# RaikoPipe/panda-gym

Hardware: AMD Instinct MI355X
Metric: aggregate env-steps/s, PandaReach 4096 envs @1 GPU; 1/2/4/8-GPU scaling (higher is better)
Workload: dtype f32; 1 GPU; PandaReach-v3 (ee control, sparse reward), 4096 envs per GPU, the reference's scene: table / plane contacts of the robot (BASELINE configs[1]); envs_per_gpu=4096, global_envs=4096, parallelism=env-sharded x1

## Files before the change

### panda-gym_amd/csrc/pgx_kernels.hip

```cpp
#include <hip/hip_runtime.h>
#include <math.h>
#include <stdint.h>

#include "../../include/pgx.h"
#include "pgx_default_model.h"
#include "pgx_common.h"
#include "pgx_dev.h"
#include "pgx_model_consts.h"
#include "pgx_rows.h"

#ifdef PGX_PROF
#define PGX_PROF_N 24
__device__ unsigned long long pgx_prof_counters[PGX_PROF_N];
#define PGX_PROF_WAVES 16384
__device__ unsigned long long pgx_prof_wave[PGX_PROF_WAVES][10];
extern "C" int pgx_prof_wave_read(unsigned long long* out, int n) {
    return (int)hipMemcpyFromSymbol(out, HIP_SYMBOL(pgx_prof_wave), sizeof(unsigned long long) * 10 * (size_t)n);
}
extern "C" int pgx_prof_read(unsigned long long* out, int clear) {
    hipError_t e = hipMemcpyFromSymbol(out, HIP_SYMBOL(pgx_prof_counters), sizeof(unsigned long long) * PGX_PROF_N);
    if (e == hipSuccess && clear) {
        unsigned long long z[PGX_PROF_N] = {0};
        e = hipMemcpyToSymbol(HIP_SYMBOL(pgx_prof_counters), z, sizeof z);
    }
// ... 287 lines not shown
}

__device__ __forceinline__ void mat_to_quat(const M3& M, float* q) {
    const float* m = M.m;
    float tr = m[0] + m[4] + m[8];
    if (tr > 0.0f) {
        float s = fast_sqrt(tr + 1.0f);
        q[3] = s * 0.5f;
        s = 0.5f * fast_rcp(s);
        q[0] = (m[7] - m[5]) * s;
        q[1] = (m[2] - m[6]) * s;
        q[2] = (m[3] - m[1]) * s;
    } else if (!(m[0] < m[4]) && !(m[0] < m[8])) {
        float s = fast_sqrt(m[0] - m[4] - m[8] + 1.0f);
        q[0] = s * 0.5f;
        s = 0.5f * fast_rcp(s);
        q[3] = (m[7] - m[5]) * s;
        q[1] = (m[3] + m[1]) * s;
        q[2] = (m[6] + m[2]) * s;
    } else if (m[0] < m[4] && !(m[4] < m[8])) {
        float s = fast_sqrt(m[4] - m[8] - m[0] + 1.0f);
        q[1] = s * 0.5f;
        s = 0.5f * fast_rcp(s);
        q[3] = (m[2] - m[6]) * s;
        q[2] = (m[7] + m[5]) * s;
        q[0] = (m[1] + m[3]) * s;
    } else {
        float s = fast_sqrt(m[8] - m[0] - m[4] + 1.0f);
        q[2] = s * 0.5f;
        s = 0.5f * fast_rcp(s);
        q[3] = (m[3] - m[1]) * s;
        q[0] = (m[2] + m[6]) * s;
        q[1] = (m[5] + m[7]) * s;
    }
}

__device__ __forceinline__ void chol7(float A[NJ][NJ]) {
#pragma unroll
    for (int j = 0; j < NJ; j++) {
        float s = A[j][j];
#pragma unroll
        for (int k = 0; k < j; k++) s -= A[j][k] * A[j][k];
        float inv = __builtin_amdgcn_rsqf(fmaxf(s, 1e-30f));
        A[j][j] = inv;
#pragma unroll
        for (int i = j + 1; i < NJ; i++) {
            float t = A[i][j];
#pragma unroll
            for (int k = 0; k < j; k++) t -= A[i][k] * A[j][k];
            A[i][j] = t * inv;
        }
    }
}
__device__ __forceinline__ void chol7_solve(const float L[NJ][NJ], const float* b, float* x) {
    float y[NJ];
#pragma unroll
    for (int i = 0; i < NJ; i++) {
        float s = b[i];
#pragma unroll
        for (int k = 0; k < i; k++) s -= L[i][k] * y[k];
        y[i] = s * L[i][i];
    }
#pragma unroll
    for (int i = NJ - 1; i >= 0; i--) {
        float s = y[i];
#pragma unroll
        for (int k = i + 1; k < NJ; k++) s -= L[k][i] * x[k];
        x[i] = s * L[i][i];
    }
}

template <bool PAR = false>
__device__ __forceinline__ void ik(MPtr mp, const float* q0, V3 target, const float* torn, float* qout) {
    float qs[NJ];
#pragma unroll
    for (int j = 0; j < NJ; j++) qs[j] = q0[j];
    float diff = 1e30f;
    const int max_iters = mp->ik_max_iters;
    const float residual = mp->ik_residual;
    for (int it = 0; it < max_iters; it++) {
        if (!(diff > residual)) break;
        PGX_PROF_COUNT(17, 1);
        MRef m = *fresh(mp);
        Chain k;
        fk_chain<PAR>(m, qs, k);
        V3 x = k.o[6] + mulc(k.R[6], kEePivot);
        M3 Ree = mulm(k.R[6], kEeRot);
        float cq[4], dq[4];
        mat_to_quat(Ree, cq);
        {
            const float ax = torn[0], ay = torn[1], az = torn[2], aw = torn[3];
            const float bx = -cq[0], by = -cq[1], bz = -cq[2], bw = cq[3];
            dq[0] = aw * bx + ax * bw + ay * bz - az * by;
            dq[1] = aw * by + ay * bw + az * bx - ax * bz;
            dq[2] = aw * bz + az * bw + ax * by - ay * bx;
            dq[3] = aw * bw - ax * bx - ay * by - az * bz;
        }
        float vn = fast_sqrt(dq[0] * dq[0] + dq[1] * dq[1] + dq[2] * dq[2]);
        float angle = 2.0f * atan2f(vn, dq[3]);
        if (angle > 3.14159265358979f) angle -= 6.28318530717959f;
        V3 axis = vn > 1e-30f ? (1.0f / vn) * v3(dq[0], dq[1], dq[2]) : v3(1.0f, 0.0f, 0.0f);
        V3 ep = target - x;
        V3 er = angle * axis;
        float A[NJ][NJ], g[NJ], dth[NJ];
        if constexpr (PAR) {
            V3 zs[NJ], os[NJ];
#pragma unroll
            for (int j = 0; j < NJ; j++) { zs[j] = col(k.R[j], 2); os[j] = k.o[j]; }
            const V3 jwc = pick_v3(zs), jvc = cross(jwc, x - pick_v3(os));
            const float gc = dot(jvc, ep) + dot(jwc, er);
            float Ac[NJ];
            sfor<0, NJ>([&](auto bc) __attribute__((always_inline)) {
                constexpr int b = decltype(bc)::value;
                const V3 jvb = v3(bcast16<b>(jvc.x), bcast16<b>(jvc.y), bcast16<b>(jvc.z));
                const V3 jwb = v3(bcast16<b>(jwc.x), bcast16<b>(jwc.y), bcast16<b>(jwc.z));
                Ac[b] = dot(jvc, jvb) + dot(jwc, jwb);
            });
            sfor<0, NJ>([&](auto ac) __attribute__((always_inline)) {
                constexpr int a = decltype(ac)::value;
                g[a] = bcast16<a>(gc);
                sfor<0, a + 1>([&](auto bc) __attribute__((always_inline)) {
                    constexpr int b = decltype(bc)::value;
                    A[a][b] = bcast16<a>(Ac[b]);
                });
                A[a][a] += m.ik_damping;
            });
        } else {
            V3 jv[NJ], jw[NJ];
#pragma unroll
            for (int j = 0; j < NJ; j++) {
                jw[j] = col(k.R[j], 2);
                jv[j] = cross(jw[j], x - k.o[j]);
            }
#pragma unroll
            for (int a = 0; a < NJ; a++) {
                g[a] = dot(jv[a], ep) + dot(jw[a], er);
#pragma unroll
                for (int b = 0; b <= a; b++) A[a][b] = dot(jv[a], jv[b]) + dot(jw[a], jw[b]);
                A[a][a] += m.ik_damping;
            }
        }
        chol7(A);
        chol7_solve(A, g, dth);
        float mx = 0.0f;
#pragma unroll
        for (int j = 0; j < NJ; j++) mx = fmaxf(mx, fabsf(dth[j]));
        float sc = mx > m.ik_max_angle ? m.ik_max_angle * fast_rcp(mx) : 1.0f;
#pragma unroll
        for (int j = 0; j < NJ; j++) qs[j] += dth[j] * sc;
        diff = norm(x - target);
    }
#pragma unroll
    for (int j = 0; j < NJ; j++) qout[j] = qs[j];
}

constexpr int AO_N = PGX_AO_OBSTACLES;
constexpr float kAoSize = 0.05f, kAoMargin = 0.001f;
constexpr float kAoCubeBound = 0.0866025404f;

__host__ __device__ constexpr int ao_slot(int c) {
    return kCapLink[c] < 0 ? -1 : (kCapLink[c] <= 7 ? kCapLink[c] : (kCapLink[c] == 9 ? 8 : -1));
}
__device__ constexpr int kAoSlot[PGX_NCAP] = {ao_slot(0), ao_slot(1), ao_slot(2), ao_slot(3), ao_slot(4),
                                              ao_slot(5), ao_slot(6), ao_slot(7), ao_slot(8), ao_slot(9),
                                              ao_slot(10), ao_slot(11), ao_slot(12), ao_slot(13)};
static_assert(PGX_NCAP == 14, "kAoSlot table");


__device__ __forceinline__ float box_sd(V3 P, V3 c, V3 h) {
    const float dx = fabsf(P.x - c.x) - h.x, dy = fabsf(P.y - c.y) - h.y, dz = fabsf(P.z - c.z) - h.z;
    const float ox = fmaxf(dx, 0.0f), oy = fmaxf(dy, 0.0f), oz = fmaxf(dz, 0.0f);
    return fast_sqrt(ox * ox + oy * oy + oz * oz) + fminf(fmaxf(dx, fmaxf(dy, dz)), 0.0f);
}

__device__ __forceinline__ V3 seg_closest(V3 A, V3 B, V3 C) {
    const V3 ab = B - A;
    const float l2 = dot(ab, ab);
    float t = l2 > 0.0f ? dot(C - A, ab) * fast_rcp(l2) : 0.0f;
    t = fminf(fmaxf(t, 0.0f), 1.0f);
    return A + t * ab;
}

__device__ __forceinline__ bool seg_meets_box(V3 A, V3 ab, V3 lo, V3 hi) {
    float t0 = 0.0f, t1 = 1.0f;
    bool miss = false;
    const float a[3] = {A.x, A.y, A.z}, d[3] = {ab.x, ab.y, ab.z}, l[3] = {lo.x, lo.y, lo.z}, u[3] = {hi.x, hi.y, hi.z};
#pragma unroll
    for (int i = 0; i < 3; i++) {
        if (fabsf(d[i]) < 1e-20f) {
            miss = miss || a[i] < l[i] || a[i] > u[i];
        } else {
            const float inv = fast_rcp(d[i]);
            const float ta = (l[i] - a[i]) * inv, tb = (u[i] - a[i]) * inv;
            t0 = fmaxf(t0, fminf(ta, tb));
            t1 = fminf(t1, fmaxf(ta, tb));
        }
// ... 1371 lines not shown
                sort_g1_by_depth(*Lp, es);
                wm = __builtin_amdgcn_readfirstlane(wm);
                while (wm) {
                    const int cn = __builtin_ctz(wm);
                    wm &= wm - 1u;
                    object_candidates_g(e, cap_tau<TAU_OBJ>(m, cn), *Lp, es, ob, Rc, cn, c, ((rm >> cn) & 1u) != 0);
                }
                PGX_PROF_MARK(21);
                sort_groups(*Lp, es);
            }
        }
    }
    PGX_PROF_MARK(1);
    const V3 g = v3(m.gravity[0], m.gravity[1], m.gravity[2]);
    const V3 base = v3(m.base[0], m.base[1], m.base[2]);
    const V3 zl = col(Rl, 2);
    const V3 ob_l = ol - base;
    const V3 cw = ol + mul(Rl, v3(K.com[0], K.com[1], K.com[2]));
    const V3 cb = cw - base;

    const float qdl = pick_arm(qd, 0.0f);
    const V3 t1 = qdl * zl;
    const V3 w = row_pre(t1);
    const V3 alt = cross(w - t1, t1);
    const V3 al = row_pre(alt);
    const V3 S = row_pre(cross(t1, ob_l));
    const V3 u = cross(w, ob_l) - S;
    const V3 dS = row_pre(cross(alt, ob_l) + cross(t1, u));
    const V3 v = cross(w, cb) - S;
    const V3 a = cross(al, cb) + cross(w, v) - dS;
    const S3 Iw = rot_sym_r(Rl, K.I);
    const V3 Iww = mul(Iw, w);
    const float wn = norm(w);
    const V3 Iow = mul(Rl, mul_sym(K.Iown, mul_t(Rl, w)));
    V3 F = K.mass * (a - g);
    V3 T = mul(Iw, al) + cross(w, Iww) + (m.ang_damp + m.ang_damp * wn) * Iow;
    {
        const V3 Fd = (K.mass * (m.lin_damp + m.lin_damp * norm(v))) * v;
        V3 Fg = v3(0, 0, 0), Tg = v3(0, 0, 0);
#pragma unroll
        for (int b = 0; b < PGX_NDAMP; b++) {
            const V3 rb = mulc(Rl, kDpos[b]);
            const V3 vb = u + cross(w, rb);
            const V3 fd = (kDmass[b] * (m.lin_damp + m.lin_damp * norm(vb))) * vb;
            Fg = Fg + fd;
            Tg = Tg + cross(ol + rb - cw, fd);
        }
        F = F + v3(lane_sel<NJ - 1>(Fg.x, Fd.x), lane_sel<NJ - 1>(Fg.y, Fd.y), lane_sel<NJ - 1>(Fg.z, Fd.z));
        T = T + v3(lane_sel<NJ - 1>(Tg.x, 0.0f), lane_sel<NJ - 1>(Tg.y, 0.0f), lane_sel<NJ - 1>(Tg.z, 0.0f));
    }
    const V3 Fs = row_suf(link_only(F));
    const V3 Ms = row_suf(link_only(T + cross(cb, F)));
    const float nbl = -dot(zl, Ms - cross(ob_l, Fs));
    float nb[NJ];
    sfor<0, NJ>([&](auto jc) __attribute__((always_inline)) {
        constexpr int j = decltype(jc)::value;
        nb[j] = bcast16<j>(nbl);
    });
    PGX_PROF_MARK(14);

    float Mt[NJ][NJ];
    {
        const float ml = link_only(K.mass);
        const S3 st = steiner(ml, cb);
        const float Mc = row_suf(ml);
        const V3 H = row_suf(ml * cb);
        const float Ixx = row_suf(link_only(Iw.xx + st.xx)), Iyy = row_suf(link_only(Iw.yy + st.yy));
        const float Izz = row_suf(link_only(Iw.zz + st.zz)), Ixy = row_suf(link_only(Iw.xy + st.xy));
        const float Ixz = row_suf(link_only(Iw.xz + st.xz)), Iyz = row_suf(link_only(Iw.yz + st.yz));
        const S3 Is = {Ixx, Iyy, Izz, Ixy, Ixz, Iyz};
        const V3 f = cross(zl, H - Mc * ob_l);
        const float Ho = dot(H, ob_l), oz = dot(ob_l, zl), Hz = dot(H, zl), oo = dot(ob_l, ob_l);
        const V3 n = mul(Is, zl) + (Mc * oo - 2.0f * Ho) * zl + oz * H + Hz * ob_l - (Mc * oz) * ob_l;
        float colv[NJ];
#pragma unroll
        for (int i = 0; i < NJ; i++) colv[i] = dot(z[i], n + cross(ol - o[i], f));
        sfor<0, NJ>([&](auto jc) __attribute__((always_inline)) {
            constexpr int j = decltype(jc)::value;
            sfor<0, j + 1>([&](auto ic) __attribute__((always_inline)) {
                constexpr int i = decltype(ic)::value;
                Mt[j][i] = bcast16<j>(colv[i]);
            });
        });
    }
    chol7(Mt);
    float (&vu)[NJ] = D.vu;
    {
        float qdd[NJ];
        chol7_solve(Mt, nb, qdd);
#pragma unroll
        for (int j = 0; j < NJ; j++) vu[j] = fminf(fmaxf(qd[j] + m.dt * qdd[j], -m.max_vel), m.max_vel);
    }

    PGX_PROF_MARK(15);
    {
        float y[NJ], x[NJ];
        sfor<0, NJ>([&](auto ic) __attribute__((always_inline)) {
            constexpr int i = decltype(ic)::value;
            float sacc = lane_sel<i>(1.0f, 0.0f);
#pragma unroll
            for (int k = 0; k < i; k++) sacc -= Mt[i][k] * y[k];
            y[i] = sacc * Mt[i][i];
        });
#pragma unroll
        for (int i = NJ - 1; i >= 0; i--) {
            float sacc = y[i];
#pragma unroll
            for (int k = i + 1; k < NJ; k++) sacc -= Mt[k][i] * x[k];
            x[i] = sacc * Mt[i][i];
        }
#pragma unroll
        for (int k = 0; k < NJ; k++) D.mcol[k] = x[k];
        sfor<0, NJ>([&](auto dc) __attribute__((always_inline)) {
            constexpr int d = decltype(dc)::value;
            D.mdiag[d] = bcast16<d>(x[d]);
        });
    }
    V3& vcu = D.vcu;
    V3& wcu = D.wcu;
    vcu = v3(0, 0, 0);
    wcu = v3(0, 0, 0);
    if (OBJ) {
        const float vn = norm(ob.v), wn2 = norm(ob.w);
        vcu = ob.v + m.dt * (g - (m.lin_damp + m.lin_damp * vn) * ob.v - cross(ob.w, ob.v));
        wcu = ob.w - (m.dt * (m.ang_damp + m.ang_damp * wn2)) * ob.w;
    }
}

__device__ __forceinline__ void object_integrate(MRef m, ObjState& ob, V3 v, V3 w) {
    ob.v = v;
    ob.w = w;
    ob.p = ob.p + m.dt * ob.v;
    float ang = norm(ob.w);
    if (ang * m.dt > 0.39269908f) ang = 0.39269908f * m.inv_dt;
    const float hdt = 0.5f * m.dt;
    const float f = ang < 0.001f ? (hdt - m.dt * m.dt * m.dt * 0.020833333333f * ang * ang)
                                 : __sinf(ang * hdt) * fast_rcp(ang);
    const float ax = ob.w.x * f, ay = ob.w.y * f, az = ob.w.z * f, aw = __cosf(ang * hdt);
    const float nx = aw * ob.qx + ax * ob.qw + ay * ob.qz - az * ob.qy;
    const float ny = aw * ob.qy + ay * ob.qw + az * ob.qx - ax * ob.qz;
    const float nz = aw * ob.qz + az * ob.qw + ax * ob.qy - ay * ob.qx;
    const float nw = aw * ob.qw - ax * ob.qx - ay * ob.qy - az * ob.qz;
// ... 392 lines not shown
            L.cache[8 + 2 * s + 1][ln] = s < n1 ? lam1[s][0] : 0.0f;
        }
    }
    if (OBJ) object_integrate(m, ob, vcu + dvl, wcu + dvw);
    PGX_PROF_MARK(5);
}

constexpr bool limit_rows_paired() {
    for (int r = 0; r < NJ; r++)
        if ((kPgxRowCode[r] >> 4) != 0) return false;
    for (int r = NJ; r + 1 < PGX_N_ROWS; r += 2)
        if ((kPgxRowCode[r] >> 4) != 1 || (kPgxRowCode[r + 1] >> 4) != 2 ||
            (kPgxRowCode[r] & 15) != (kPgxRowCode[r + 1] & 15))
            return false;
    return (PGX_N_ROWS - NJ) % 2 == 0;
}

constexpr int last_motor_row() {
    int r = 0;
    for (int i = 0; i < PGX_N_ROWS; i++)
        if ((kPgxRowCode[i] >> 4) == 0) r = i;
    return r;
}

template <int OBJ, int CONT, int PART = 1, int AO = 0, int FULL = 0>
__device__ __forceinline__ bool substep_g(MPtr mp, const PgxDevEnv& e, float* q, float* qd, const float* tq,
                                          ObjState& ob, ContactLdsGT<OBJ, FULL>* Lp, int es, int c, const LaneK& K,
                                          bool check = false) {
    MRef m = *fresh(mp);
    constexpr bool LDS_LIM = OBJ;
    constexpr bool NO_PART = OBJ && PART == 2;
    constexpr bool PERS = CONT && FULL && (OBJ || (AO && AO_PERS));
    Dyn D;
    substep_dyn_g<OBJ, CONT, AO, FULL>(m, e, q, qd, ob, Lp, es, D, c, K, check);
    if constexpr (AO) {
        if (D.coll) return true;
    }
    const V3 (&z)[NJ] = D.z;
    const V3 (&o)[NJ] = D.o;
    float vu[NJ];
#pragma unroll
    for (int j = 0; j < NJ; j++) vu[j] = D.vu[j];
    V3 vcu = D.vcu, wcu = D.wcu;
    PGX_PROF_MARK(2);
    const bool arm = c < NJ;
    const float inv_m = e.obj_inv_mass, inv_i = e.obj_inv_inertia;
    float mcol[NJ];
#pragma unroll
    for (int d = 0; d < NJ; d++) mcol[d] = D.mcol[d];
    const float kobj = OBJ ? ((c >= 7 && c < 10) ? inv_m : ((c >= 10 && c < 13) ? inv_i : 0.0f)) : 0.0f;
    const float vu_c = pick_gen(vu, vcu, wcu);
    float gv = 0.0f;

    constexpr int P0 = OBJ ? CG : 0;
    constexpr int CGR = ContactLdsGT<OBJ, FULL>::CGR;
    constexpr int NP = P0 + (CONT ? CGR : 0);
    constexpr int RB = CONT ? ContactLdsGT<OBJ, FULL>::RB : CGR;
    constexpr int NQR = ContactLdsGT<OBJ, FULL>::NQR;
    constexpr int NC_ = OBJ ? 13 : NJ;
    constexpr int XSTEP = 1;
    int n1x = 0;
    int nxr = 0;
    float cJ[NP > 0 ? NP : 1][3], cR[NP > 0 ? NP : 1][3], crhs[NP > 0 ? NP : 1][3], cjinv[NP > 0 ? NP : 1][3];
    float cden[NP > 0 ? NP : 1][3], clam[NP > 0 ? NP : 1][3];
    float pmu[NP > 0 ? NP : 1];
    bool act[NP > 0 ? NP : 1];
    int n0 = 0, n1 = 0;
    if (CONT) {
        ContactLdsGT<OBJ, FULL>& L = *Lp;
        n0 = L.cnt[0][es];
        n1 = L.cnt[1][es];
        const float erp_dt = m.contact_erp * m.inv_dt;
        float cid0[CG], cim0[CG], cid1[CGR], cim1[CGR];
#pragma unroll
        for (int s2 = 0; s2 < CG; s2++) {
            cid0[s2] = OBJ ? L.cache[2 * s2][es] : -1.0f;
            cim0[s2] = OBJ ? L.cache[2 * s2 + 1][es] : 0.0f;
        }
#pragma unroll
        for (int s2 = 0; s2 < CGR; s2++) {
            cid1[s2] = L.cache[CACHE1 + 2 * s2][es];
            cim1[s2] = L.cache[CACHE1 + 2 * s2 + 1][es];
        }
        auto warm_of = [&](const float* ids, const float* ims, auto n_c, float id) __attribute__((always_inline)) {
            float w = 0.0f;
#pragma unroll
            for (int s2 = 0; s2 < decltype(n_c)::value; s2++) w = ids[s2] == id ? m.warmstart * ims[s2] : w;
            return w;
        };
#pragma unroll
        for (int p = 0; p < NP; p++) pmu[p] = m.friction;
#pragma unroll
        for (int k = 0; k < P0; k++) {
            act[k] = k < n0;
            const float4 r4 = L.g0q[k][0][es];
            const V3 r = v3(r4.x, r4.y, r4.z);
            const float id = L.g0id[k][es];
            const float warm = warm_of(cid0, cim0, IC<CG>{}, id);
            V3 nk = lds3(L.g0n[k], es), t1, t2;
            nk = act[k] ? nk : v3(0.0f, 0.0f, 1.0f);
            plane_space(nk, t1, t2);
#pragma unroll
            for (int dir = 0; dir < 3; dir++) {
                const V3 lin = dir == 0 ? nk : (dir == 1 ? t1 : t2);
                const V3 ang = cross(r, lin);
                const float den = inv_m + dot(ang, ang) * inv_i;
                const float jinv = den > 2.220446e-16f ? fast_rcp(den) : 0.0f;
                const float rel = dot(lin, vcu) + dot(ang, wcu);
                float rhs;
                if (dir == 0) {
                    const float pen = L.g0d[k][es];
                    rhs = (pen > 0.0f ? (-rel - pen * m.inv_dt) : (-pen * erp_dt - rel)) * jinv;
                } else {
                    rhs = -rel * jinv;
                }
                const float J = pick_obj(lin, ang);
                cJ[k][dir] = act[k] ? J : 0.0f;
                cR[k][dir] = act[k] ? J * kobj : 0.0f;
                crhs[k][dir] = act[k] ? rhs : 0.0f;
                cjinv[k][dir] = act[k] ? jinv : 0.0f;
                cden[k][dir] = act[k] ? den : 0.0f;
                clam[k][dir] = (act[k] && dir == 0) ? warm : 0.0f;
                gv += cR[k][dir] * clam[k][dir];
            }
        }
        const V3 zc = pick_v3(z), oc = pick_v3(o);
        V3 gP[CGR], gN[CGR], gRb[CGR];
        int gJ[CGR], gW[CGR];
        float gId[CGR], gD[CGR];
        auto read_point = [&](int k) __attribute__((always_inline)) {
            gP[k] = v3(L.g1p[k][0][es], L.g1p[k][1][es], L.g1p[k][2][es]);
            gN[k] = v3(L.g1n[k][0][es], L.g1n[k][1][es], L.g1n[k][2][es]);
            gRb[k] = OBJ ? v3(L.g1rb[k][0][es], L.g1rb[k][1][es], L.g1rb[k][2][es]) : v3(0.0f, 0.0f, 0.0f);
            gJ[k] = L.g1j[k][es];
            gW[k] = PERS ? L.g1w[k][es] : -1;
            gId[k] = L.g1id[k][es];
            gD[k] = L.g1d[k][es];
        };
        auto warm_pt = [&](int w, float id) __attribute__((always_inline)) {
            return (PERS && w >= 0) ? m.warmstart * L.mimp[w < 0 ? 0 : w][es] : warm_of(cid1, cim1, IC<CGR>{}, id);
        };
        if (!AO && __any(n1 > 0)) {
#pragma unroll
            for (int k = 0; k < CGR; k++) read_point(k);
        }
#pragma unroll
        for (int k = 0; k < (CONT ? CGR : 0); k++) {
            const int p = P0 + k;
            act[p] = k < n1;
#pragma unroll
            for (int dir = 0; dir < 3; dir++) {
                cJ[p][dir] = 0.0f; cR[p][dir] = 0.0f; crhs[p][dir] = 0.0f;
                cjinv[p][dir] = 0.0f; cden[p][dir] = 0.0f; clam[p][dir] = 0.0f;
            }
            if (__any(act[p])) {
                if (AO) read_point(k);
                const V3 P = gP[k];
                const V3 n = gN[k];
                const V3 rb = gRb[k];
                const int jl = gJ[k];
                const float id = gId[k];
                pmu[p] = point_mu<AO, FULL>(m, id);
                const bool vs_obj = OBJ && id >= kTableIdLimit;
                const float warm = warm_pt(gW[k], id);
                V3 t1, t2;
                plane_space(n, t1, t2);
                const V3 Jv = (arm && c <= jl) ? cross(zc, P - oc) : v3(0, 0, 0);
#pragma unroll
                for (int dir = 0; dir < 3; dir++) {
                    const V3 u = dir == 0 ? n : (dir == 1 ? t1 : t2);
                    float J = dot(u, Jv);
                    if (OBJ) {
                        const V3 ca = cross(rb, u);
                        const float oj = pick_obj(-1.0f * u, -1.0f * ca);
                        J = (!arm && vs_obj) ? oj : J;
                    }
                    float R = kobj * J;
                    sfor<0, NJ>([&](auto bc) __attribute__((always_inline)) {
                        constexpr int b = decltype(bc)::value;
                        R += mcol[b] * bcast16<b>(J);
                    });
                    const float den = sum16(J * R);
                    const float rel = sum16(J * vu_c);
                    const float jinv = den > 2.220446e-16f ? fast_rcp(den) : 0.0f;
                    float rhs;
                    if (dir == 0) {
                        const float pen = gD[k];
                        rhs = (pen > 0.0f ? (-rel - pen * m.inv_dt) : (-pen * erp_dt - rel)) * jinv;
                    } else {
                        rhs = -rel * jinv;
                    }
                    cJ[p][dir] = act[p] ? J : 0.0f;
                    cR[p][dir] = act[p] ? R : 0.0f;
// ... 173 lines not shown
    PGX_PROF_MARK(23);

    float den[NJ], jinv[NJ];
#pragma unroll
    for (int d = 0; d < NJ; d++) {
        den[d] = D.mdiag[d];
        jinv[d] = den[d] > 2.220446e-16f ? fast_rcp(den[d]) : 0.0f;
    }
    float rhs[PGX_N_ROWS];
#pragma unroll
    for (int r = 0; r < PGX_N_ROWS; r++) {
        const int kind = kPgxRowCode[r] >> 4, d = kPgxRowCode[r] & 15;
        rhs[r] = 0.0f;
        if (kind == 0) {
            const float pos_term = (tq[d] - q[d]) * m.inv_dt;
            const float desired = m.kp * pos_term + vu[d] + m.kd * (0.0f - vu[d]);
            rhs[r] = desired - vu[d];
        }
    }
    auto init_limit_rows = [&]() __attribute__((always_inline)) {
#pragma unroll
        for (int r = 0; r < PGX_N_ROWS; r++) {
            const int kind = kPgxRowCode[r] >> 4, d = kPgxRowCode[r] & 15;
            if (kind == 0) continue;
            const float rel = kind == 2 ? -vu[d] : vu[d];
            const float pen = kind == 1 ? (q[d] - kLower[d]) : (kUpper[d] - q[d]);
            float verr = -rel, perr = 0.0f;
            if (pen > 0.0f) verr -= pen * m.inv_dt;
            else perr = -pen * m.erp * m.inv_dt;
            rhs[r] = perr + verr;
        }
    };
    bool ok_c = true;
    bool far_nc = true;
    if (arm) {
        float B = 0.0f;
#pragma unroll
        for (int k = 0; k < NJ; k++) B += fabsf(mcol[k]) * m.max_impulse[k];
        B = B * 1.001f + 1e-6f;
        float lo_a[NJ], up_a[NJ];
#pragma unroll
        for (int d = 0; d < NJ; d++) { lo_a[d] = kLower[d]; up_a[d] = kUpper[d]; }
        const float qc = pick_arm(q, 0.0f);
        const float penl = qc - pick_arm(lo_a, 0.0f), penu = pick_arm(up_a, 0.0f) - qc;
        ok_c = penl > 0.0f && penu > 0.0f && (vu_c - B) > -penl * m.inv_dt && (vu_c + B) < penu * m.inv_dt;
    }
    far_nc = !row_any(!ok_c);
    const bool far = far_nc && n1 == 0;
    float mcs[NJ], wms[NJ], wms2[NJ];
    constexpr int PK = AO ? PGX_PK_AO : PGX_PK;
    constexpr bool PKM = WROWS && (PK & 1) != 0, PKC = WROWS && (PK & 2) != 0;
    constexpr bool PKD = TWO && FULL && !PKM && !PKC && (PK & 4) != 0;
    constexpr bool MERGE = WROWS && !OBJ && !AO && !PKM && !PKC && PART != 2;
    constexpr int MG0 = 8;
    static_assert(!MERGE || MG0 + 6 <= GW, "6 contact rows from lane MG0");
    auto hi_sel = [&](float a, float other) __attribute__((always_inline)) {
        float r;
        asm("v_cndmask_b32 %0, %1, %2, %3" : "=v"(r) : "v"(other), "v"(a), "s"(0xFF00FF00FF00FF00ull));
        return r;
    };
    auto ror8 = [&](float v) __attribute__((always_inline)) { return dpp<0x128>(v); };
    f2 mw[NJ], crw[NQ], mw2[NJ], cw2[NQ];
    f2 bnd[NJ];
    float lam[PGX_N_ROWS], lhi[NJ];
#pragma unroll
    for (int d = 0; d < NJ; d++) {
        mcs[d] = mcol[d] * jinv[d];
        wms[d] = Wm[d] * jinv[d];
        wms2[d] = Wm2[d] * jinv[d];
        lhi[d] = m.limit_max_imp * den[d];
    }
    auto init_bounds = [&]() __attribute__((always_inline)) {
#pragma unroll
        for (int r = 0; r < PGX_N_ROWS; r++) {
            const int kind = kPgxRowCode[r] >> 4, d = kPgxRowCode[r] & 15;
            lam[r] = 0.0f;
            if (kind == 0) bnd[d] = (f2){-m.max_impulse[d] * den[d], m.max_impulse[d] * den[d]};
            else if (LDS_LIM) __hip_atomic_store(&Lp->llam[r - NJ][es], 0.0f, __ATOMIC_RELAXED, __HIP_MEMORY_SCOPE_WAVEFRONT);
        }
    };
    init_bounds();
    auto mrow = [&](auto rc, auto g2_c, auto mg_c, float& resid) __attribute__((always_inline)) {
        constexpr int r = decltype(rc)::value;
        constexpr int kind = kPgxRowCode[r] >> 4, d = kPgxRowCode[r] & 15;
        const float x = kind == 2 ? rhs[r] + bcast16<d>(gv) : rhs[r] - bcast16<d>(gv);
        float delta;
        if constexpr (kind == 0) {
            delta = __builtin_amdgcn_fmed3f(x, bnd[d].x, bnd[d].y);
            bnd[d] -= (f2){delta, delta};
        } else if constexpr (LDS_LIM) {
            float* lr = &Lp->lrhs[r - NJ][es];
            float* ll = &Lp->llam[r - NJ][es];
            const float rr = __hip_atomic_load(lr, __ATOMIC_RELAXED, __HIP_MEMORY_SCOPE_WAVEFRONT);
            const float lm = __hip_atomic_load(ll, __ATOMIC_RELAXED, __HIP_MEMORY_SCOPE_WAVEFRONT);
            const float xl = kind == 2 ? rr + bcast16<d>(gv) : rr - bcast16<d>(gv);
            delta = __builtin_amdgcn_fmed3f(xl, -lm, lhi[d] - lm);
            __hip_atomic_store(ll, lm + delta, __ATOMIC_RELAXED, __HIP_MEMORY_SCOPE_WAVEFRONT);
        } else {
            delta = __builtin_amdgcn_fmed3f(x, -lam[r], lhi[d] - lam[r]);
            lam[r] += delta;
        }
        const float sd = kind == 2 ? -delta : delta;
        if constexpr (decltype(mg_c)::value) {
            gv += mcs[d] * sd;
        } else if constexpr (PKD) {
            gv += mcs[d] * sd;
// ... 237 lines not shown
        if constexpr (TWO && decltype(g2_c)::value) gw2 += swms2[S] * sd;
        if constexpr (decltype(mg_c)::value == 2) resid = fabsf(delta);
        else resid = fmaxf(resid, fabsf(delta));
    };
    static_assert(limit_rows_paired(), "limit rows come as (lower, upper) pairs of one dof after the motor rows");
    auto solve = [&](auto mode_c, auto nw_c, auto k_c, auto nx_c, auto mg_c) __attribute__((always_inline)) {
        constexpr int MODE = decltype(mode_c)::value;
        constexpr int NW = decltype(nw_c)::value;
        constexpr int K = decltype(k_c)::value;
        constexpr bool G2 = TWO && (NW < 0 || 3 * (P0 + NW) > GW);
        const IC<G2 ? 1 : 0> g2_c{};
        constexpr bool MG = decltype(mg_c)::value != 0;
        const IC<MG ? 2 : 0> mgf_c{};
        constexpr int LASTM = last_motor_row();
        for (int it = 0; it < n_it; it += 2) {
            float resid = 0.0f;
            if constexpr (MODE == 1 || MODE == 3) limit_check();
            if constexpr (MODE == 3) {
                sfor<0, K>([&](auto i) __attribute__((always_inline)) {
                    constexpr int S = K - 1 - decltype(i)::value;
                    if constexpr (MG && S == K - 1) srow(IC<S>{}, IC<2>{}, g2_c, mgf_c, resid);
                    else srow(IC<S>{}, IC<2>{}, g2_c, mg_c, resid);
                    srow(IC<S>{}, IC<1>{}, g2_c, mg_c, resid);
                    limit_check();
                });
            }
            sfor<0, PGX_N_ROWS>([&](auto i) __attribute__((always_inline)) {
                constexpr int r = PGX_N_ROWS - 1 - decltype(i)::value;
                if constexpr (MG && MODE != 3 && r == LASTM) mrow(IC<r>{}, g2_c, mgf_c, resid);
                else if constexpr (MODE == 2 || (kPgxRowCode[r] >> 4) == 0) mrow(IC<r>{}, g2_c, mg_c, resid);
            });
            if (CONT && (OBJ || NW > 0 || (NW < 0 && any_contact))) contact_rows(nw_c, nx_c, g2_c, mg_c, resid);
            PGX_PROF_SWEEP();
            if (resid <= res_thr || it + 1 >= n_it) break;
            resid = 0.0f;
            sfor<0, PGX_N_ROWS>([&](auto i) __attribute__((always_inline)) {
                constexpr int r = decltype(i)::value;
                if constexpr (MG && r == 0) mrow(IC<r>{}, g2_c, mgf_c, resid);
                else if constexpr (MODE == 2 || (kPgxRowCode[r] >> 4) == 0) mrow(IC<r>{}, g2_c, mg_c, resid);
            });
            if constexpr (MODE == 1 || MODE == 3) limit_check();
            if constexpr (MODE == 3) {
                sfor<0, K>([&](auto sc) __attribute__((always_inline)) {
                    srow(sc, IC<1>{}, g2_c, mg_c, resid);
                    srow(sc, IC<2>{}, g2_c, mg_c, resid);
                    limit_check();
                });
            }
            if (CONT && (OBJ || NW > 0 || (NW < 0 && any_contact))) contact_rows(nw_c, nx_c, g2_c, mg_c, resid);
            PGX_PROF_SWEEP();
            if (resid <= res_thr) break;
        }
    };
    const bool mg = MERGE && e.pgs_mode != 4 && n1w >= 1 && n1w <= 2 && nxr == 0;
    auto merge_rows = [&]() __attribute__((always_inline)) {
        if constexpr (MERGE) {
#pragma unroll
            for (int d = 0; d < NJ; d++) mcs[d] = hi_sel(ror8(wms[d]), mcs[d]);
#pragma unroll
            for (int q = 0; q < 6; q++) cR[q / 3][q % 3] = hi_sel(ror8(Wc[q]), cR[q / 3][q % 3]);
            gv = hi_sel(ror8(gw), gv);
        }
    };
    auto split_rows = [&]() __attribute__((always_inline)) {
        if constexpr (MERGE) {
#pragma unroll
            for (int d = 0; d < NJ; d++) wms[d] = hi_sel(0.0f, ror8(mcs[d]));
#pragma unroll
            for (int q = 0; q < 6; q++) Wc[q] = hi_sel(0.0f, ror8(cR[q / 3][q % 3]));
        }
    };
    auto solve_w = [&](auto mode_c, auto k_c, auto mgi_c) __attribute__((always_inline)) {
        constexpr int MODE = decltype(mode_c)::value;
        const IC<0> m0{};
        if constexpr (decltype(mgi_c)::value) {
            solve(mode_c, IC<2>{}, k_c, IC<0>{}, IC<(MODE != 2) ? 1 : 0>{});
        } else if constexpr (WROWS) {
            if (n1w == 0) solve(mode_c, IC<0>{}, k_c, IC<0>{}, m0);
            else if (nxr == 0 && n1w <= 2) solve(mode_c, IC<2>{}, k_c, IC<0>{}, m0);
            else if (CGR > 4 && nxr == 0 && n1w <= 4) solve(mode_c, IC<(CGR > 4 ? 4 : CGR)>{}, k_c, IC<0>{}, m0);
            else if constexpr (RB > CGR && MODE != 3) {
                if (nxr == 0) {
                    solve(mode_c, IC<CGR>{}, k_c, IC<0>{}, m0);
                } else {
                    sfor<1, (RB - CGR) / XSTEP + 1>([&](auto ic) __attribute__((always_inline)) {
                        constexpr int NXC = decltype(ic)::value * XSTEP;
                        if (nxr == NXC) solve(mode_c, IC<CGR>{}, k_c, IC<NXC>{}, m0);
                    });
                }
            } else {
                solve(mode_c, IC<CGR>{}, k_c, IC<0>{}, m0);
            }
        } else {
            solve(mode_c, IC<-1>{}, k_c, IC<0>{}, m0);
        }
    };
#ifndef PGX_NO_PARK_SOLVE
    constexpr bool PARK_SOLVE = CONT && (OBJ || AO || PART == 2);
#else
    constexpr bool PARK_SOLVE = false;
#endif
    auto park = [&](int k, float v) __attribute__((always_inline)) {
        __hip_atomic_store(&Lp->psv[k][es], v, __ATOMIC_RELAXED, __HIP_MEMORY_SCOPE_WAVEFRONT);
    };
    auto unpark = [&](int k) __attribute__((always_inline)) {
        return __hip_atomic_load(&Lp->psv[k][es], __ATOMIC_RELAXED, __HIP_MEMORY_SCOPE_WAVEFRONT);
    };
    if constexpr (PARK_SOLVE) {
#pragma unroll
        for (int j = 0; j < NJ; j++) { park(j, q[j]); park(NJ + j, vu[j]); }
        if constexpr (OBJ) {
            park(14, ob.p.x); park(15, ob.p.y); park(16, ob.p.z);
            park(17, ob.qx); park(18, ob.qy); park(19, ob.qz); park(20, ob.qw);
            park(21, vcu.x); park(22, vcu.y); park(23, vcu.z);
            park(24, wcu.x); park(25, wcu.y); park(26, wcu.z);
        }
    }
    if (__all(far)) {
        solve(IC<0>{}, IC<0>{}, IC<0>{}, IC<0>{}, IC<0>{});
    } else {
        PGX_PROF_COUNT(10, 1);
        init_limit_rows();
        if constexpr (LDS_LIM) {
#pragma unroll
            for (int r = NJ; r < PGX_N_ROWS; r++)
                __hip_atomic_store(&Lp->lrhs[r - NJ][es], rhs[r], __ATOMIC_RELAXED, __HIP_MEMORY_SCOPE_WAVEFRONT);
        }
        if (e.pgs_mode != 2) {
            float rl[NJ], ru[NJ];
#pragma unroll
            for (int r = NJ; r < PGX_N_ROWS; r++) {
                const int kind = kPgxRowCode[r] >> 4, d = kPgxRowCode[r] & 15;
                if (kind == 1) rl[d] = rhs[r];
                else ru[d] = rhs[r];
            }
            rl_c = pick_arm(rl, -3.0e38f);
            ru_c = pick_arm(ru, -3.0e38f);
            const bool spec_all = __all(far_nc);
            int nk = 0;
            if (!spec_all) {
                const uint64_t bm = __ballot(arm && !ok_c);
                dmask = __builtin_amdgcn_readfirstlane((unsigned)((bm | (bm >> 16) | (bm >> 32) | (bm >> 48)) & 0x7Fu));
                nk = __builtin_popcount(dmask);
            }
            const float gv0 = gv, gw0 = gw, gw20 = gw2;
            if constexpr (CONT) {
#pragma unroll
                for (int p = 0; p < NP; p++) Lp->pl0[p][es] = clam[p][0];
            }
            if constexpr (MERGE) {
                auto limit_solves = [&](auto mgi_c) __attribute__((always_inline)) {
#include "pgx_limit_solves.inc"
                };
                if (mg) limit_solves(IC<1>{});
                else limit_solves(IC<0>{});
            } else {
                const IC<0> mgi_c{};
#include "pgx_limit_solves.inc"
            }
        } else {
            PGX_PROF_COUNT(13, 1);
            solve_w(IC<2>{}, IC<0>{}, IC<0>{});
        }
    }
    PGX_PROF_SWEEPS_DONE();
    PGX_PROF_MARK(4);
    PGX_PROF_COUNT(11, any_contact ? 1 : 0);
    if constexpr (PARK_SOLVE) {
#pragma unroll
        for (int j = 0; j < NJ; j++) { q[j] = unpark(j); vu[j] = unpark(NJ + j); }
        if constexpr (OBJ) {
            ob.p = v3(unpark(14), unpark(15), unpark(16));
            ob.qx = unpark(17); ob.qy = unpark(18); ob.qz = unpark(19); ob.qw = unpark(20);
            vcu = v3(unpark(21), unpark(22), unpark(23));
            wcu = v3(unpark(24), unpark(25), unpark(26));
        }
    }
    sfor<0, NJ>([&](auto jc) __attribute__((always_inline)) {
        constexpr int j = decltype(jc)::value;
        const float vn = fminf(fmaxf(vu[j] + bcast16<j>(gv), -m.max_vel), m.max_vel);
        qd[j] = vn;
        q[j] += m.dt * vn;
    });
    if (CONT) {
        ContactLdsGT<OBJ, FULL>& L = *Lp;
        float gid0[CG], pj0[CG], gid1[CGR], pj1[CGR];
#pragma unroll
        for (int s = 0; s < CG; s++) {
            gid0[s] = OBJ ? L.g0id[s][es] : -1.0f;
            pj0[s] = OBJ ? L.pjn[s][es] : 0.0f;
        }
#pragma unroll
        for (int s = 0; s < CGR; s++) {
            gid1[s] = L.g1id[s][es];
            pj1[s] = L.pjn[P0 + s][es];
        }
#pragma unroll
        for (int s = 0; s < CG; s++) {
            L.cache[2 * s][es] = (OBJ && s < n0) ? gid0[s] : -1.0f;
            L.cache[2 * s + 1][es] = (OBJ && s < n0) ? clam[s][0] * pj0[s] : 0.0f;
        }
#pragma unroll
        for (int s = 0; s < CGR; s++) {
            L.cache[CACHE1 + 2 * s][es] = s < n1 ? gid1[s] : -1.0f;
            L.cache[CACHE1 + 2 * s + 1][es] = s < n1 ? clam[P0 + s][0] * pj1[s] : 0.0f;
        }
        if constexpr (RB > CGR) {
            if (n1x > CGR) {
#pragma unroll
                for (int b = 0; b < XB; b++)
                    if (GW * b + c < 3 * (n1x - CGR)) L.xlam[GW * b + c][es] = xs_lam[b];
                __builtin_amdgcn_fence(__ATOMIC_SEQ_CST, "wavefront");
            }
            for (int s = CGR; s < RB; s++) {
                const int xq = 3 * (s - CGR);
                L.cache[CACHE1 + 2 * s][es] = s < n1 ? L.g1id[s][es] : -1.0f;
                L.cache[CACHE1 + 2 * s + 1][es] = s < n1 ? L.xlam[xq][es] * L.xjinv[xq][es] : 0.0f;
            }
        }
        if constexpr (PERS) {
            static_assert(RB <= GW, "one lane per robot slot");
            __builtin_amdgcn_fence(__ATOMIC_SEQ_CST, "wavefront");
            if (c < n1) {
                const int w = L.g1w[c][es];
                if (w >= 0) L.mimp[w][es] = L.cache[CACHE1 + 2 * c + 1][es];
            }
        }
    }
    if (OBJ) {
        const V3 dvl = v3(bcast16<7>(gv), bcast16<8>(gv), bcast16<9>(gv));
        const V3 dvw = v3(bcast16<10>(gv), bcast16<11>(gv), bcast16<12>(gv));
        object_integrate(m, ob, vcu + dvl, wcu + dvw);
    }
    PGX_PROF_MARK(5);
    return false;
}

__device__ __forceinline__ void ee_state(MRef m, const float* q, const float* qd, V3& pos, V3& vel) {
    Chain k;
    fk_chain(m, q, k);
    pos = k.o[NJ - 1] + mulc(k.R[NJ - 1], kEeCom);
    V3 vv = v3(0, 0, 0);
#pragma unroll
    for (int j = 0; j < NJ; j++) vv = vv + qd[j] * cross(col(k.R[j], 2), pos - k.o[j]);
    vel = vv;
}

__device__ __forceinline__ void ee_state_cached(MRef m, const float* qc, const float* q, const float* qd, V3& pos,
                                                V3& vel) {
    Chain k;
    fk_chain(m, q, k);
    const V3 p = k.o[NJ - 1] + mulc(k.R[NJ - 1], kEeCom);
    V3 vv = v3(0, 0, 0);
#pragma unroll
    for (int j = 0; j < NJ; j++) vv = vv + qd[j] * cross(col(k.R[j], 2), p - k.o[j]);
    const V3 vl = mul_t(k.R[NJ - 1], vv);
    Chain kc;
    fk_chain(m, qc, kc);
    pos = kc.o[NJ - 1] + mulc(kc.R[NJ - 1], kEeCom);
    vel = mul(kc.R[NJ - 1], vl);
}

constexpr uint32_t TAG_RESET = 0x52455345u;
constexpr uint32_t TAG_ACTION = 0x41435430u;

__device__ __forceinline__ double reset_uniform_s(uint64_t seed, uint64_t env, uint32_t episode, int kidx) {
    uint32_t o[4];
    philox((uint32_t)env, (uint32_t)(env >> 32), episode, TAG_RESET + (uint32_t)(kidx >> 1), (uint32_t)seed,
           (uint32_t)(seed >> 32), o);
    uint64_t u = (kidx & 1) ? ((uint64_t)o[2] | ((uint64_t)o[3] << 32)) : ((uint64_t)o[0] | ((uint64_t)o[1] << 32));
    return (double)(u >> 11) * (1.0 / 9007199254740992.0);
}
__device__ __forceinline__ double reset_uniform(const PgxDevEnv& e, uint64_t env, uint32_t episode, int kidx) {
    return reset_uniform_s(e.seed, env, episode, kidx);
}

struct Pcg64 {
    uint64_t lo, hi, ilo, ihi;
    uint32_t has, u32;
};
__device__ __forceinline__ Pcg64 pcg64_load(const uint64_t* r) {
// ... 1486 lines not shown
```

Baseline: 11.73 million env-steps/s.

## Fuse Cholesky factor with forward solve and specialize two-point contact path

Adds a lane-parallel Cholesky routine that factors the row-distributed matrix and does the forward substitution in the same pass. It replaces the broadcast-to-full-matrix, factor and separate solve steps in the parallel IK branch and in the mass-matrix dynamics step. The contact solve section is wrapped in a lambda instantiated twice: a two-contact-point specialization taken when no env in the wave has more than two robot contacts, and a general fallback. This aims to cut register pressure and work in the common case, at the cost of more code size and extra stores that clear unused cache slots.

Result: faster. 12.21 million env-steps/s (median of 6 runs) (+4.1%).

```diff
diff --git a/panda-gym_amd/csrc/pgx_kernels.hip b/panda-gym_amd/csrc/pgx_kernels.hip
--- a/panda-gym_amd/csrc/pgx_kernels.hip
+++ b/panda-gym_amd/csrc/pgx_kernels.hip
@@ -363,6 +363,15 @@
         }
     }
 }
+__device__ __forceinline__ void chol7_back(const float L[NJ][NJ], const float* y, float* x) {
+#pragma unroll
+    for (int i = NJ - 1; i >= 0; i--) {
+        float s = y[i];
+#pragma unroll
+        for (int k = i + 1; k < NJ; k++) s -= L[k][i] * x[k];
+        x[i] = s * L[i][i];
+    }
+}
 __device__ __forceinline__ void chol7_solve(const float L[NJ][NJ], const float* b, float* x) {
     float y[NJ];
 #pragma unroll
@@ -372,13 +381,32 @@
         for (int k = 0; k < i; k++) s -= L[i][k] * y[k];
         y[i] = s * L[i][i];
     }
-#pragma unroll
-    for (int i = NJ - 1; i >= 0; i--) {
-        float s = y[i];
-#pragma unroll
-        for (int k = i + 1; k < NJ; k++) s -= L[k][i] * x[k];
-        x[i] = s * L[i][i];
-    }
+    chol7_back(L, y, x);
+}
+__device__ __forceinline__ void chol7_rows(float* a, float b, float L[NJ][NJ], float* y) {
+    sfor<0, NJ>([&](auto jc) __attribute__((always_inline)) {
+        constexpr int j = decltype(jc)::value;
+        float t = a[j];
+        sfor<0, j>([&](auto kc) __attribute__((always_inline)) {
+            constexpr int k = decltype(kc)::value;
+            t -= a[k] * bcast16<j>(a[k]);
+        });
+        const float inv = __builtin_amdgcn_rsqf(fmaxf(bcast16<j>(t), 1e-30f));
+        L[j][j] = inv;
+        a[j] = t * inv;
+    });
+    sfor<0, NJ>([&](auto ic) __attribute__((always_inline)) {
+        constexpr int i = decltype(ic)::value;
+        sfor<0, i>([&](auto kc) __attribute__((always_inline)) {
+            constexpr int k = decltype(kc)::value;
+            L[i][k] = bcast16<i>(a[k]);
+        });
+    });
+    sfor<0, NJ>([&](auto kc) __attribute__((always_inline)) {
+        constexpr int k = decltype(kc)::value;
+        y[k] = bcast16<k>(b) * L[k][k];
+        b -= a[k] * y[k];
+    });
 }
 
 template <bool PAR = false>
@@ -427,15 +455,12 @@
                 const V3 jwb = v3(bcast16<b>(jwc.x), bcast16<b>(jwc.y), bcast16<b>(jwc.z));
                 Ac[b] = dot(jvc, jvb) + dot(jwc, jwb);
             });
-            sfor<0, NJ>([&](auto ac) __attribute__((always_inline)) {
-                constexpr int a = decltype(ac)::value;
-                g[a] = bcast16<a>(gc);
-                sfor<0, a + 1>([&](auto bc) __attribute__((always_inline)) {
-                    constexpr int b = decltype(bc)::value;
-                    A[a][b] = bcast16<a>(Ac[b]);
-                });
-                A[a][a] += m.ik_damping;
+            sfor<0, NJ>([&](auto bc) __attribute__((always_inline)) {
+                constexpr int b = decltype(bc)::value;
+                Ac[b] += lane_sel<b>(m.ik_damping, -0.0f);
             });
+            chol7_rows(Ac, gc, A, g);
+            chol7_back(A, g, dth);
         } else {
             V3 jv[NJ], jw[NJ];
 #pragma unroll
@@ -450,9 +475,9 @@
                 for (int b = 0; b <= a; b++) A[a][b] = dot(jv[a], jv[b]) + dot(jw[a], jw[b]);
                 A[a][a] += m.ik_damping;
             }
-        }
-        chol7(A);
-        chol7_solve(A, g, dth);
+            chol7(A);
+            chol7_solve(A, g, dth);
+        }
         float mx = 0.0f;
 #pragma unroll
         for (int j = 0; j < NJ; j++) mx = fmaxf(mx, fabsf(dth[j]));
@@ -1930,14 +1955,9 @@
     const V3 Fs = row_suf(link_only(F));
     const V3 Ms = row_suf(link_only(T + cross(cb, F)));
     const float nbl = -dot(zl, Ms - cross(ob_l, Fs));
-    float nb[NJ];
-    sfor<0, NJ>([&](auto jc) __attribute__((always_inline)) {
-        constexpr int j = decltype(jc)::value;
-        nb[j] = bcast16<j>(nbl);
-    });
     PGX_PROF_MARK(14);
 
-    float Mt[NJ][NJ];
+    float Mt[NJ][NJ], yb[NJ];
     {
         const float ml = link_only(K.mass);
         const S3 st = steiner(ml, cb);
@@ -1953,19 +1973,12 @@
         float colv[NJ];
 #pragma unroll
         for (int i = 0; i < NJ; i++) colv[i] = dot(z[i], n + cross(ol - o[i], f));
-        sfor<0, NJ>([&](auto jc) __attribute__((always_inline)) {
-            constexpr int j = decltype(jc)::value;
-            sfor<0, j + 1>([&](auto ic) __attribute__((always_inline)) {
-                constexpr int i = decltype(ic)::value;
-                Mt[j][i] = bcast16<j>(colv[i]);
-            });
-        });
-    }
-    chol7(Mt);
+        chol7_rows(colv, nbl, Mt, yb);
+    }
     float (&vu)[NJ] = D.vu;
     {
         float qdd[NJ];
-        chol7_solve(Mt, nb, qdd);
+        chol7_back(Mt, yb, qdd);
 #pragma unroll
         for (int j = 0; j < NJ; j++) vu[j] = fminf(fmaxf(qd[j] + m.dt * qdd[j], -m.max_vel), m.max_vel);
     }
@@ -2464,10 +2477,29 @@
     const float vu_c = pick_gen(vu, vcu, wcu);
     float gv = 0.0f;
 
+    constexpr int CGR_ALL = ContactLdsGT<OBJ, FULL>::CGR;
+    constexpr bool MERGE_K = CONT && !OBJ && !AO && ((AO ? PGX_PK_AO : PGX_PK) & 3) == 0 && PART != 2;
+#ifndef PGX_CONTACT_INPLACE
+#if defined(PGX_TU) && (PGX_TU == 2 || PGX_TU == 4)
+#define PGX_CONTACT_INPLACE 1
+#else
+#define PGX_CONTACT_INPLACE 0
+#endif
+#endif
+#if PGX_CONTACT_INPLACE
+    static_assert(!MERGE_K, "a kernel that merges needs the instances (not PGX_CONTACT_INPLACE)");
+    const IC<CGR_ALL> cgr_c{};
+    {
+#else
+    auto contact_part = [&](auto cgr_c) __attribute__((always_inline)) {
+#endif
     constexpr int P0 = OBJ ? CG : 0;
-    constexpr int CGR = ContactLdsGT<OBJ, FULL>::CGR;
+    constexpr int CGR = decltype(cgr_c)::value;
+    constexpr bool TWOPT = CGR < CGR_ALL;
+    static_assert(!TWOPT || (MERGE_K && CGR == 2), "the two-point instance belongs to the kernels that merge");
     constexpr int NP = P0 + (CONT ? CGR : 0);
-    constexpr int RB = CONT ? ContactLdsGT<OBJ, FULL>::RB : CGR;
+    constexpr int RB_ALL = CONT ? ContactLdsGT<OBJ, FULL>::RB : CGR_ALL;
+    constexpr int RB = TWOPT ? CGR : RB_ALL;
     constexpr int NQR = ContactLdsGT<OBJ, FULL>::NQR;
     constexpr int NC_ = OBJ ? 13 : NJ;
     constexpr int XSTEP = 1;
@@ -2483,14 +2515,14 @@
         n0 = L.cnt[0][es];
         n1 = L.cnt[1][es];
         const float erp_dt = m.contact_erp * m.inv_dt;
-        float cid0[CG], cim0[CG], cid1[CGR], cim1[CGR];
+        float cid0[CG], cim0[CG], cid1[CGR_ALL], cim1[CGR_ALL];
 #pragma unroll
         for (int s2 = 0; s2 < CG; s2++) {
             cid0[s2] = OBJ ? L.cache[2 * s2][es] : -1.0f;
             cim0[s2] = OBJ ? L.cache[2 * s2 + 1][es] : 0.0f;
         }
 #pragma unroll
-        for (int s2 = 0; s2 < CGR; s2++) {
+        for (int s2 = 0; s2 < CGR_ALL; s2++) {
             cid1[s2] = L.cache[CACHE1 + 2 * s2][es];
             cim1[s2] = L.cache[CACHE1 + 2 * s2 + 1][es];
         }
@@ -2550,7 +2582,7 @@
             gD[k] = L.g1d[k][es];
         };
         auto warm_pt = [&](int w, float id) __attribute__((always_inline)) {
-            return (PERS && w >= 0) ? m.warmstart * L.mimp[w < 0 ? 0 : w][es] : warm_of(cid1, cim1, IC<CGR>{}, id);
+            return (PERS && w >= 0) ? m.warmstart * L.mimp[w < 0 ? 0 : w][es] : warm_of(cid1, cim1, IC<CGR_ALL>{}, id);
         };
         if (!AO && __any(n1 > 0)) {
 #pragma unroll
@@ -2830,6 +2862,7 @@
     constexpr bool PKM = WROWS && (PK & 1) != 0, PKC = WROWS && (PK & 2) != 0;
     constexpr bool PKD = TWO && FULL && !PKM && !PKC && (PK & 4) != 0;
     constexpr bool MERGE = WROWS && !OBJ && !AO && !PKM && !PKC && PART != 2;
+    static_assert(MERGE == MERGE_K, "MERGE_K (the instances' choice) restates MERGE");
     constexpr int MG0 = 8;
     static_assert(!MERGE || MG0 + 6 <= GW, "6 contact rows from lane MG0");
     auto hi_sel = [&](float a, float other) __attribute__((always_inline)) {
@@ -3173,7 +3206,7 @@
             if (resid <= res_thr) break;
         }
     };
-    const bool mg = MERGE && e.pgs_mode != 4 && n1w >= 1 && n1w <= 2 && nxr == 0;
+    const bool mg = TWOPT && n1w >= 1;
     auto merge_rows = [&]() __attribute__((always_inline)) {
         if constexpr (MERGE) {
 #pragma unroll
@@ -3196,6 +3229,9 @@
         const IC<0> m0{};
         if constexpr (decltype(mgi_c)::value) {
             solve(mode_c, IC<2>{}, k_c, IC<0>{}, IC<(MODE != 2) ? 1 : 0>{});
+        } else if constexpr (TWOPT) {
+            if (MODE != 2 || n1w == 0) solve(mode_c, IC<0>{}, k_c, IC<0>{}, m0);
+            else solve(mode_c, IC<2>{}, k_c, IC<0>{}, m0);
         } else if constexpr (WROWS) {
             if (n1w == 0) solve(mode_c, IC<0>{}, k_c, IC<0>{}, m0);
             else if (nxr == 0 && n1w <= 2) solve(mode_c, IC<2>{}, k_c, IC<0>{}, m0);
@@ -3273,8 +3309,12 @@
                 auto limit_solves = [&](auto mgi_c) __attribute__((always_inline)) {
 #include "pgx_limit_solves.inc"
                 };
-                if (mg) limit_solves(IC<1>{});
-                else limit_solves(IC<0>{});
+                if constexpr (TWOPT) {
+                    if (mg) limit_solves(IC<1>{});
+                    else limit_solves(IC<0>{});
+                } else {
+                    limit_solves(IC<0>{});
+                }
             } else {
                 const IC<0> mgi_c{};
 #include "pgx_limit_solves.inc"
@@ -3339,6 +3379,13 @@
                 L.cache[CACHE1 + 2 * s + 1][es] = s < n1 ? L.xlam[xq][es] * L.xjinv[xq][es] : 0.0f;
             }
         }
+        if constexpr (TWOPT) {
+#pragma unroll
+            for (int s = CGR; s < RB_ALL; s++) {
+                L.cache[CACHE1 + 2 * s][es] = -1.0f;
+                L.cache[CACHE1 + 2 * s + 1][es] = 0.0f;
+            }
+        }
         if constexpr (PERS) {
             static_assert(RB <= GW, "one lane per robot slot");
             __builtin_amdgcn_fence(__ATOMIC_SEQ_CST, "wavefront");
@@ -3348,6 +3395,18 @@
             }
         }
     }
+#if PGX_CONTACT_INPLACE
+    }
+#else
+    };
+    if constexpr (MERGE_K) {
+        const bool two = e.pgs_mode != 4 && !__any(Lp->cnt[1][es] > 2);
+        if (two) contact_part(IC<2>{});
+        else contact_part(IC<CGR_ALL>{});
+    } else {
+        contact_part(IC<CGR_ALL>{});
+    }
+#endif
     if (OBJ) {
         const V3 dvl = v3(bcast16<7>(gv), bcast16<8>(gv), bcast16<9>(gv));
         const V3 dvw = v3(bcast16<10>(gv), bcast16<11>(gv), bcast16<12>(gv));
```
